# tusen-ai/SST

Hardware: AMD Instinct MI355X
Metric: LiDAR frames/sec (SST backbone fwd+bwd) at Waymo 0.32m voxels (higher is better)
Workload: dtype f32 (storage, accumulation, attention, LayerNorm, reductions: fp32; the dense products of the encoder layers from the EXACT three-way bf16 split of both fp32 operands, six bf16 MFMA products with fp32 accumulation - error vs float64 <= 2 x the fp32 matrix pipe's: tests/test_gpu_dense_f32x6.py)

## Files before the change

sst_amd/csrc/dense_f32x6.hip:

```cpp
#include <math.h>
#include <stdlib.h>
#include "common.h"
#include "tile_io.h"

namespace {

typedef float f32x4 __attribute__((ext_vector_type(4)));
typedef float f32x2 __attribute__((ext_vector_type(2)));
typedef unsigned u32x4 __attribute__((ext_vector_type(4)));
typedef __bf16 bf16x8 __attribute__((ext_vector_type(8)));
typedef __bf16 bf16x2 __attribute__((ext_vector_type(2)));

__device__ __forceinline__ unsigned pack2(float lo, float hi) {
  const f32x2 v = {lo, hi};
  return __builtin_bit_cast(unsigned, __builtin_convertvector(v, bf16x2));
}
__device__ __forceinline__ float lo_f(unsigned p) { return __uint_as_float(p << 16); }
__device__ __forceinline__ float hi_f(unsigned p) { return __uint_as_float(p & 0xffff0000u); }
__device__ __forceinline__ f32x4 mma32(u32x4 a, u32x4 b, f32x4 c) {
  return __builtin_amdgcn_mfma_f32_16x16x32_bf16(__builtin_bit_cast(bf16x8, a), __builtin_bit_cast(bf16x8, b), c, 0, 0, 0);
}
__device__ __forceinline__ void split2(float a, float b, unsigned& p0, unsigned& p1, unsigned& p2) {
  p0 = pack2(a, b);
  const float ra = a - lo_f(p0), rb = b - hi_f(p0);
// ... 3 lines not shown
__device__ __forceinline__ void split8(const f32x4& a, const f32x4& b, u32x4& p0, u32x4& p1, u32x4& p2) {
  unsigned q0[4], q1[4], q2[4];
  split2(a[0], a[1], q0[0], q1[0], q2[0]);
  split2(a[2], a[3], q0[1], q1[1], q2[1]);
  split2(b[0], b[1], q0[2], q1[2], q2[2]);
  split2(b[2], b[3], q0[3], q1[3], q2[3]);
  p0 = (u32x4){q0[0], q0[1], q0[2], q0[3]};
  p1 = (u32x4){q1[0], q1[1], q1[2], q1[3]};
  p2 = (u32x4){q2[0], q2[1], q2[2], q2[3]};
}

__device__ __forceinline__ float erf_as(float z, float& e) {
  const float az = fabsf(z);
  const float t = __builtin_amdgcn_rcpf(fmaf(0.3275911f, az, 1.f));
  e = __expf(-az * az);
  const float poly = t * fmaf(t, fmaf(t, fmaf(t, fmaf(t, 1.061405429f, -1.453152027f), 1.421413741f), -0.284496736f), 0.254829592f);
  return copysignf(fmaf(-poly, e, 1.f), z);
}
__device__ __forceinline__ float gelu_f(float x) {
  float e;
  return 0.5f * x * (1.f + erf_as(x * 0.70710678118654752f, e));
}
__device__ __forceinline__ float gelu_grad_f(float x) {
  float e;
  const float phi = 0.5f * (1.f + erf_as(x * 0.70710678118654752f, e));
  return fmaf(x * 0.3989422804014327f, e, phi);
}

enum { kEpiBias = 0, kEpiGelu = 1, kEpiRelu = 2, kEpiMulGeluGrad = 3, kEpiMulReluGrad = 4, kEpiAdd = 5, kEpiAddLN = 6,
       kEpiAddRows = 7 };

struct ln_epi {
  const float* w;
  const float* b;
  float eps;
  float2* stats;
  const float* pos_table;
  const int32_t* pos_idx;
  float* yp;
};

__device__ __forceinline__ int w_lds_row(int n) {
  const int tp = n >> 5, within = n & 31;
  return 16 * (2 * tp + ((within >> 2) & 1)) + ((within >> 3) << 2) + (within & 3);
}

template <int K, int NW, int EPI>
constexpr bool x6_bias_in_regs() {
  return 3 * NW * K * 2 + NW * (EPI == kEpiAddLN ? 3 : 1) * 4 + 8 * 2048 > 160 * 1024;
}
template <int K, int NW, int EPI>
constexpr int x6_lds_bytes() {
  return 3 * NW * K * 2 + (x6_bias_in_regs<K, NW, EPI>() ? 0 : NW * (EPI == kEpiAddLN ? 3 : 1) * 4) + 8 * 2048;
}

template <int K, int NW, int EPI, bool XADD = false>
__global__ __launch_bounds__(512, 2) void tall_linear_f32x6_k(
    const float* __restrict__ X, const float* __restrict__ X2, int x2_from, int64_t ldx, const float* __restrict__ W,
    int64_t ldw, int trans_w, const float* __restrict__ bias, int64_t M, int row_blocks, int rows_per_wave,
    float* __restrict__ Y, int64_t ldy, const float* __restrict__ aux_in, float* __restrict__ aux_out, int64_t ldaux,
    const ln_epi ln, const float* __restrict__ xadd_rows = nullptr, const int32_t* __restrict__ xadd_idx = nullptr) {
  static_assert(EPI != kEpiAddLN || NW == 128, "the LayerNorm epilogue needs a whole 128-wide row in one accumulator set");
  static_assert(NW == 64 || NW == 128, "column group");
  constexpr int KS = K / 32, NTH = 512, TILES = NW / 16, EMITS = TILES / 2;
  constexpr int IMG = NW * K * 2;
  constexpr bool BIAS_REG = x6_bias_in_regs<K, NW, EPI>();
  constexpr bool HAS_AUX = EPI == kEpiMulGeluGrad || EPI == kEpiMulReluGrad || EPI == kEpiAdd || EPI == kEpiAddLN || EPI == kEpiAddRows;
  static_assert(!(BIAS_REG && EPI == kEpiAddLN), "the LayerNorm epilogue reads its row parameters from LDS");
  extern __shared__ __attribute__((aligned(16))) unsigned char smem6[];
  unsigned char* w0 = smem6;
  unsigned char* w1 = smem6 + IMG;
  unsigned char* w2 = smem6 + 2 * IMG;
  float* bimg = (float*)(smem6 + 3 * IMG);
  auto frag_off = [](int lr, int k8) { return ((lr >> 4) * KS + (k8 >> 5)) * 1024 + (16 * ((k8 >> 3) & 3) + (lr & 15)) * 16; };
  const int lane = threadIdx.x & 63, g = lane >> 4, c = lane & 15;
  const int wv = __builtin_amdgcn_readfirstlane(threadIdx.x >> 6);
  const int rr = lane >> 3, rcol = (lane & 7) * 4;
  const tile_xpose io =
      make_tile_xpose(smem6 + 3 * IMG + (BIAS_REG ? 0 : NW * (EPI == kEpiAddLN ? 3 : 1) * 4) + wv * 2048, lane);
  const int grp = blockIdx.x / row_blocks, rb = blockIdx.x - grp * row_blocks;
  const int nb = grp * NW;
  const float* __restrict__ Xg = grp >= x2_from ? X2 : X;
  const int64_t wave = (int64_t)rb * 8 + wv;
  int64_t r0 = wave * rows_per_wave;
  const int64_t r1 = r0 + rows_per_wave < M ? r0 + rows_per_wave : M;
  auto row_of = [&](int64_t r, int i) {
    const int64_t row = r + 8 * i + rr;
    return row < M ? row : M - 1;
  };
  constexpr int D = EPI == kEpiAddLN ? 2 : (KS > 8 ? KS / 2 : KS);
  static_assert(!XADD || D == KS, "the positional rows of a tile are requested with one set of indices");
  static_assert(KS % D == 0, "a block keeps its slot from tile to tile");
  f32x4 xr[D][2];
  auto issue_x = [&](int64_t r, int s) {
#pragma unroll
    for (int i = 0; i < 2; ++i) xr[s % D][i] = *(const f32x4*)(Xg + row_of(r, i) * ldx + 32 * s + rcol);
  };
  const bool xadd = XADD && grp < x2_from;
  f32x4 pr[XADD ? D : 1][2];
  int32_t pi[2] = {0, 0};
  auto load_pidx = [&](int64_t r, int32_t (&dst)[2]) {
#pragma unroll
    for (int i = 0; i < 2; ++i) dst[i] = xadd_idx[row_of(r, i)];
  };
  auto issue_p = [&](int s) {
#pragma unroll
// ... 138 lines not shown
            pend[T][r] -= mean;
            sq = fmaf(pend[T][r], pend[T][r], sq);
          }
        sq += __shfl_xor(sq, 16, 64);
        sq += __shfl_xor(sq, 32, 64);
        ln_rstd = rsqrtf(sq * (1.f / 128.f) + ln.eps);
        if (g == 0 && pend_r0 + c < M) ln.stats[pend_r0 + c] = make_float2(mean, ln_rstd);
      }
      const int n0 = 32 * tp + 8 * g;
      const f32x4 y0 = pend[2 * tp] * ln_rstd * *(const f32x4*)(bimg + NW + n0) + *(const f32x4*)(bimg + 2 * NW + n0);
      const f32x4 y1 =
          pend[2 * tp + 1] * ln_rstd * *(const f32x4*)(bimg + NW + n0 + 4) + *(const f32x4*)(bimg + 2 * NW + n0 + 4);
      f32x4 t[2];
      tile_to_rows(io, y0, y1, t[0], t[1]);
#pragma unroll
      for (int i = 0; i < 2; ++i)
        if (pv[i]) *(f32x4*)(Y + prow[i] * ldy + 32 * tp + rcol) = t[i];
      if (gather) {
#pragma unroll
        for (int i = 0; i < 2; ++i)
          if (pv[i]) *(f32x4*)(ln.yp + prow[i] * 128 + 32 * tp + rcol) = t[i] + qr[i];
      }
      return;
    }
    const int n0 = nb + 32 * tp + rcol;
    const f32x4 bv = BIAS_REG ? breg[BIAS_REG ? tp : 0] : *(const f32x4*)(bimg + 32 * tp + rcol);
    f32x4 t[2];
    tile_to_rows(io, pend[2 * tp], pend[2 * tp + 1], t[0], t[1]);
#pragma unroll
    for (int i = 0; i < 2; ++i) {
      f32x4 v = t[i] + bv;
      if (EPI == kEpiGelu || EPI == kEpiRelu) {
        if (aux_out != nullptr && pv[i]) *(f32x4*)(aux_out + prow[i] * ldaux + n0) = v;
#pragma unroll
        for (int r = 0; r < 4; ++r) v[r] = EPI == kEpiGelu ? gelu_f(v[r]) : fmaxf(v[r], 0.f);
      }
      if (EPI == kEpiMulGeluGrad || EPI == kEpiMulReluGrad) {
        const f32x4 p = ar[HAS_AUX ? tp : 0][i];
#pragma unroll
        for (int r = 0; r < 4; ++r) v[r] *= EPI == kEpiMulGeluGrad ? gelu_grad_f(p[r]) : (p[r] > 0.f ? 1.f : 0.f);
      }
      if (EPI == kEpiAdd || EPI == kEpiAddRows) v += ar[HAS_AUX ? tp : 0][i];
      if (pv[i]) *(f32x4*)(Y + prow[i] * ldy + n0) = v;
    }
  };
  auto emit = [&](int tp, bool in_loop) {
    if (pend_valid) consume(tp);
    if (in_loop)
      request(tp);
    else if (EPI == kEpiAddLN && gather && tp + 1 < EMITS)
      issue_q(ep, tp + 1);
  };

  for (; r0 < r1; r0 += 16) {
    asm volatile("" ::: "memory");
    const int64_t rn = r0 + 16 < r1 ? r0 + 16 : r0;
    int32_t pj[2] = {0, 0};
    if (xadd) load_pidx(r0 + 32, pj);
    if (GATHER && gather) load_eidx(r0 + 16, en);
    f32x4 acc[TILES];
#pragma unroll
    for (int T = 0; T < TILES; ++T) acc[T] = (f32x4){0.f, 0.f, 0.f, 0.f};
    constexpr int QPS = TILES / 4;
    constexpr int G = KS * QPS;
    u32x4 x0, x1, x2;
#pragma clang loop unroll(full)
    for (int q = 0; q < G; ++q) {
      const int s = q / QPS, t0 = (q % QPS) * 4;
      if (q % QPS == 0) {
        f32x4 a = xr[s % D][0], b = xr[s % D][1];
        if (XADD && xadd) {
          a += pr[XADD ? s % D : 0][0];
          b += pr[XADD ? s % D : 0][1];
        }
        f32x4 v0, v1;
        tile_to_frag(io, a, b, v0, v1);
        split8(v0, v1, x0, x1, x2);
        if (s + D < KS) {
          issue_x(r0, s + D);
        } else {
          issue_x(rn, s + D - KS);
          if (XADD && xadd) issue_p(s + D - KS);
        }
        __builtin_amdgcn_sched_barrier(0x786);
      }
      u32x4 a0[4], a1[4], a2[4];
#pragma unroll
      for (int u = 0; u < 4; ++u) {
        const int off = lane_off + ((t0 + u) * KS + s) * 1024;
        a0[u] = *(const u32x4*)(w0 + off);
        a1[u] = *(const u32x4*)(w1 + off);
        a2[u] = *(const u32x4*)(w2 + off);
      }
#pragma unroll
      for (int u = 0; u < 4; ++u) acc[t0 + u] = mma32(a0[u], x2, acc[t0 + u]);
#pragma unroll
      for (int u = 0; u < 4; ++u) acc[t0 + u] = mma32(a2[u], x0, acc[t0 + u]);
#pragma unroll
      for (int u = 0; u < 4; ++u) acc[t0 + u] = mma32(a1[u], x1, acc[t0 + u]);
#pragma unroll
      for (int u = 0; u < 4; ++u) acc[t0 + u] = mma32(a0[u], x1, acc[t0 + u]);
#pragma unroll
      for (int u = 0; u < 4; ++u) acc[t0 + u] = mma32(a1[u], x0, acc[t0 + u]);
#pragma unroll
      for (int u = 0; u < 4; ++u) acc[t0 + u] = mma32(a0[u], x0, acc[t0 + u]);
      if ((q + 1) % (G / EMITS) == 0) emit((q + 1) / (G / EMITS) - 1, true);
    }
#pragma unroll
    for (int T = 0; T < TILES; ++T) pend[T] = acc[T];
    pend_r0 = r0;
    pend_valid = true;
#pragma unroll
    for (int i = 0; i < 2; ++i) {
      pi[i] = pj[i];
      ep[i] = ec[i];
      ec[i] = en[i];
    }
  }
#pragma unroll
  for (int tp = 0; tp < EMITS; ++tp) emit(tp, false);
}

void x6_partition(int64_t m, int groups, int64_t& row_blocks, int64_t& rpw) {
  row_blocks = (256 / groups) & ~7;
  rpw = sst_align_up(sst_div_up(m, row_blocks * 8), 16);
  row_blocks = sst_align_up(sst_div_up(m, rpw * 8), 8);
}

template <int K, int NW, int EPI, bool XADD = false>
int launch_x6(const float* x, const float* x2, int x2_from, int64_t ldx, const float* w, int64_t ldw, int trans_w,
              const float* bias, int64_t m, int n, float* y, int64_t ldy, const float* aux_in, float* aux_out, int64_t ldaux,
              hipStream_t st, const ln_epi ln = ln_epi(), const float* xadd_rows = nullptr, const int32_t* xadd_idx = nullptr) {
  constexpr int lds = x6_lds_bytes<K, NW, EPI>();
  static_assert(lds <= 160 * 1024, "three weight images of a column group and the waves' blocks must fit the CU's LDS");
  static unsigned long long configured = 0;
  if (sst_first_use_on_device(&configured)) {
    SST_HIP(hipFuncSetAttribute((const void*)tall_linear_f32x6_k<K, NW, EPI, XADD>, hipFuncAttributeMaxDynamicSharedMemorySize, lds));
    sst_mark_device(&configured);
  }
  const int groups = n / NW;
  int64_t row_blocks, rpw;
  x6_partition(m, groups, row_blocks, rpw);
  if (x2 == nullptr) x2_from = groups;
  hipLaunchKernelGGL((tall_linear_f32x6_k<K, NW, EPI, XADD>), dim3((unsigned)(row_blocks * groups)), dim3(512), lds, st, x, x2,
                     x2_from, ldx, w, ldw, trans_w, bias, m, (int)row_blocks, (int)rpw, y, ldy, aux_in, aux_out, ldaux, ln, xadd_rows,
                     xadd_idx);
  return SST_OK;
}

template <int K, int NW>
int dispatch_x6(int epi, const float* x, const float* x2, int x2_from, int64_t ldx, const float* w, int64_t ldw, int trans_w,
                const float* bias, int64_t m, int n, float* y, int64_t ldy, const float* aux_in, float* aux_out, int64_t ldaux,
                hipStream_t st) {
#define SST_CASE(E) \
  case E: return launch_x6<K, NW, E>(x, x2, x2_from, ldx, w, ldw, trans_w, bias, m, n, y, ldy, aux_in, aux_out, ldaux, st)
  switch (epi) {
    SST_CASE(kEpiBias);
    SST_CASE(kEpiGelu);
    SST_CASE(kEpiRelu);
// ... 131 lines not shown
```

sst_amd/csrc/layer_tail_x6.hip:

```cpp
#include <math.h>
#include <stdlib.h>
#include "common.h"

#ifndef SST_NT_OUT
#define SST_NT_OUT false
#endif
#ifndef SST_NT_BWD
#define SST_NT_BWD true
#endif

namespace {

typedef float f32x4 __attribute__((ext_vector_type(4)));
typedef float f32x2 __attribute__((ext_vector_type(2)));
typedef unsigned u32x4 __attribute__((ext_vector_type(4)));
typedef __bf16 bf16x8 __attribute__((ext_vector_type(8)));
typedef __bf16 bf16x2 __attribute__((ext_vector_type(2)));

__device__ __forceinline__ unsigned pack2(float lo, float hi) {
  const f32x2 v = {lo, hi};
  return __builtin_bit_cast(unsigned, __builtin_convertvector(v, bf16x2));
}
__device__ __forceinline__ float lo_f(unsigned p) { return __uint_as_float(p << 16); }
__device__ __forceinline__ float hi_f(unsigned p) { return __uint_as_float(p & 0xffff0000u); }
// ... 206 lines not shown
__device__ __forceinline__ void barrier_lds_only() { asm volatile("s_waitcnt lgkmcnt(0)\n\ts_barrier" ::: "memory"); }
__device__ __forceinline__ void barrier_drain() { asm volatile("s_waitcnt vmcnt(0) lgkmcnt(0)\n\ts_barrier" ::: "memory"); }

struct tile_io {
  unsigned char* scr;
  int frag_off0;
  int row_off[2];
  int64_t rrow[2];
  bool rvalid[2];
  int rcol;
};
__device__ __forceinline__ tile_io make_tile_io(unsigned char* scr, int lane, int64_t r0, int64_t m) {
  tile_io t;
  const int c = lane & 15, g = lane >> 4;
  t.scr = scr;
  t.frag_off0 = c * 128 + (((2 * g) ^ (c & 7)) << 4);
#pragma unroll
  for (int i = 0; i < 2; ++i) {
    const int r = 8 * i + (lane >> 3), p = lane & 7;
    t.row_off[i] = r * 128 + ((p ^ (r & 7)) << 4);
    t.rvalid[i] = r0 + r < m;
    t.rrow[i] = t.rvalid[i] ? r0 + r : m - 1;
  }
  t.rcol = (lane & 7) * 4;
  return t;
}
template <bool STREAM>
__device__ __forceinline__ void store32(const tile_io& t, float* __restrict__ base, int64_t ld, int col0, const f32x4& v0,
                                        const f32x4& v1) {
  *(f32x4*)(t.scr + t.frag_off0) = v0;
  *(f32x4*)(t.scr + (t.frag_off0 ^ 16)) = v1;
#pragma unroll
  for (int i = 0; i < 2; ++i) {
    const f32x4 w = *(const f32x4*)(t.scr + t.row_off[i]);
    if (t.rvalid[i]) {
      if (STREAM)
        __builtin_nontemporal_store(w, (f32x4*)(base + t.rrow[i] * ld + col0 + t.rcol));
      else
        *(f32x4*)(base + t.rrow[i] * ld + col0 + t.rcol) = w;
    }
  }
}
__device__ __forceinline__ void load32_issue(const tile_io& t, const float* __restrict__ base, int64_t ld, int col0, f32x4 (&w)[2]) {
#pragma unroll
  for (int i = 0; i < 2; ++i) w[i] = *(const f32x4*)(base + t.rrow[i] * ld + col0 + t.rcol);
}
__device__ __forceinline__ void load32_finish(const tile_io& t, const f32x4 (&w)[2], f32x4& v0, f32x4& v1) {
#pragma unroll
  for (int i = 0; i < 2; ++i) *(f32x4*)(t.scr + t.row_off[i]) = w[i];
  v0 = *(const f32x4*)(t.scr + t.frag_off0);
  v1 = *(const f32x4*)(t.scr + (t.frag_off0 ^ 16));
}

template <int HALF>
__device__ __forceinline__ void mma_half(const unsigned char* slot, int lane_off, const f32x4 (&x)[4][2], f32x4 (&acc)[8]) {
#pragma unroll
  for (int s2 = 0; s2 < 2; ++s2) {
    const img3 xs = split8(x[2 * HALF + s2][0], x[2 * HALF + s2][1]);
#pragma unroll
    for (int t0 = 0; t0 < 8; t0 += 4) {
      u32x4 a0[4], a1[4], a2[4];
#pragma unroll
      for (int u = 0; u < 4; ++u) {
        const int off = lane_off + ((t0 + u) * 2 + s2) * kFrag;
        a0[u] = *(const u32x4*)(slot + off);
        a1[u] = *(const u32x4*)(slot + kIA + off);
        a2[u] = *(const u32x4*)(slot + 2 * kIA + off);
      }
#pragma unroll
      for (int u = 0; u < 4; ++u) acc[t0 + u] = mma32(a0[u], xs.p2, acc[t0 + u]);
#pragma unroll
      for (int u = 0; u < 4; ++u) acc[t0 + u] = mma32(a2[u], xs.p0, acc[t0 + u]);
#pragma unroll
      for (int u = 0; u < 4; ++u) acc[t0 + u] = mma32(a1[u], xs.p1, acc[t0 + u]);
#pragma unroll
      for (int u = 0; u < 4; ++u) acc[t0 + u] = mma32(a0[u], xs.p1, acc[t0 + u]);
#pragma unroll
      for (int u = 0; u < 4; ++u) acc[t0 + u] = mma32(a1[u], xs.p0, acc[t0 + u]);
#pragma unroll
      for (int u = 0; u < 4; ++u) acc[t0 + u] = mma32(a0[u], xs.p0, acc[t0 + u]);
    }
  }
}

__device__ __forceinline__ f32x4 add4(const f32x4& a, const f32x4& b) {
  return (f32x4){a[0] + b[0], a[1] + b[1], a[2] + b[2], a[3] + b[3]};
}

__device__ __forceinline__ void mma_first(const unsigned char* slot, int lane_off1, const img3 (&y)[4], f32x4& out0, f32x4& out1) {
  const f32x4 z = {0.f, 0.f, 0.f, 0.f};
  f32x4 am[2] = {z, z}, ca[2] = {z, z}, cb[2] = {z, z};
#pragma unroll
  for (int s = 0; s < 4; ++s) {
    u32x4 a0[2], a1[2], a2[2];
#pragma unroll
    for (int T = 0; T < 2; ++T) {
      const int off = lane_off1 + (T * 4 + s) * kFrag;
      a0[T] = *(const u32x4*)(slot + off);
      a1[T] = *(const u32x4*)(slot + kI1 + off);
      a2[T] = *(const u32x4*)(slot + 2 * kI1 + off);
    }
#pragma unroll
    for (int T = 0; T < 2; ++T) ca[T] = mma32(a0[T], y[s].p2, ca[T]);
#pragma unroll
    for (int T = 0; T < 2; ++T) cb[T] = mma32(a0[T], y[s].p1, cb[T]);
#pragma unroll
    for (int T = 0; T < 2; ++T) ca[T] = mma32(a2[T], y[s].p0, ca[T]);
#pragma unroll
    for (int T = 0; T < 2; ++T) am[T] = mma32(a0[T], y[s].p0, am[T]);
#pragma unroll
    for (int T = 0; T < 2; ++T) ca[T] = mma32(a1[T], y[s].p1, ca[T]);
#pragma unroll
    for (int T = 0; T < 2; ++T) cb[T] = mma32(a1[T], y[s].p0, cb[T]);
  }
  out0 = add4(am[0], add4(cb[0], ca[0]));
  out1 = add4(am[1], add4(cb[1], ca[1]));
}

__device__ __forceinline__ void mma_second(const unsigned char* slot2, int lane_off2, const img3& h, f32x4 (&acc)[8]) {
#pragma unroll
  for (int t0 = 0; t0 < 8; t0 += 4) {
    u32x4 a0[4], a1[4], a2[4];
#pragma unroll
    for (int u = 0; u < 4; ++u) {
      const int off = lane_off2 + (t0 + u) * kFrag;
      a0[u] = *(const u32x4*)(slot2 + off);
      a1[u] = *(const u32x4*)(slot2 + kI2 + off);
      a2[u] = *(const u32x4*)(slot2 + 2 * kI2 + off);
    }
#pragma unroll
    for (int u = 0; u < 4; ++u) acc[t0 + u] = mma32(a0[u], h.p2, acc[t0 + u]);
#pragma unroll
    for (int u = 0; u < 4; ++u) acc[t0 + u] = mma32(a2[u], h.p0, acc[t0 + u]);
#pragma unroll
    for (int u = 0; u < 4; ++u) acc[t0 + u] = mma32(a1[u], h.p1, acc[t0 + u]);
#pragma unroll
    for (int u = 0; u < 4; ++u) acc[t0 + u] = mma32(a0[u], h.p1, acc[t0 + u]);
#pragma unroll
    for (int u = 0; u < 4; ++u) acc[t0 + u] = mma32(a1[u], h.p0, acc[t0 + u]);
#pragma unroll
    for (int u = 0; u < 4; ++u) acc[t0 + u] = mma32(a0[u], h.p0, acc[t0 + u]);
  }
}

__device__ __forceinline__ void ln_stats(f32x4 (&v)[4][2], float eps, float& mean, float& rstd) {
  float sum = 0.f;
#pragma unroll
  for (int s = 0; s < 4; ++s)
#pragma unroll
    for (int r = 0; r < 4; ++r) sum += v[s][0][r] + v[s][1][r];
  sum += __shfl_xor(sum, 16, 64);
  sum += __shfl_xor(sum, 32, 64);
  mean = sum * (1.f / 128.f);
  float sq = 0.f;
#pragma unroll
  for (int s = 0; s < 4; ++s)
#pragma unroll
    for (int h = 0; h < 2; ++h)
#pragma unroll
      for (int r = 0; r < 4; ++r) {
        v[s][h][r] -= mean;
        sq = fmaf(v[s][h][r], v[s][h][r], sq);
      }
  sq += __shfl_xor(sq, 16, 64);
  sq += __shfl_xor(sq, 32, 64);
  rstd = rsqrtf(sq * (1.f / 128.f) + eps);
}

struct tail_fwd_params {
  const float *o, *x;
  const unsigned char* packed;
  const float *b_out, *b1, *b2, *n1w, *n1b, *n2w, *n2b;
  float eps;
  int64_t m;
  float *s1, *st1, *y1, *pre, *h, *s2, *st2, *y2;
  const float* pos_table;
  const int32_t* pos_idx;
  float* y2p;
};

template <int ACT>
__global__ __launch_bounds__(kNTH, 2) void encoder_tail_fwd_x6_k(const tail_fwd_params P) {
  extern __shared__ __attribute__((aligned(16))) unsigned char lds[];
  float* par = (float*)(lds + kArea);
  const int lane = threadIdx.x & 63, g = lane >> 4, c = lane & 15, wave = threadIdx.x >> 6;
  const int64_t r0 = (int64_t)blockIdx.x * kRowsPerWg + wave * 16;
  const bool valid = r0 + c < P.m;
  const int64_t row = valid ? r0 + c : P.m - 1;
  const tile_io io = make_tile_io(lds + kArea + kParF * 4 + wave * kScr, lane, r0, P.m);
  const unsigned char* packed = P.packed;
  unsigned char* const part2 = lds + kPart1;
  dma_pieces(packed, lds, 3 * kIA / 1024, wave, lane);
  f32x4 ob[4][2], xr[4][2];
  {
    f32x4 wo[4][2], wx[4][2];
#pragma unroll
    for (int s = 0; s < 4; ++s) load32_issue(io, P.o, kC, 32 * s, wo[s]);
#pragma unroll
    for (int s = 0; s < 4; ++s) load32_issue(io, P.x, kC, 32 * s, wx[s]);
#pragma unroll
    for (int s = 0; s < 4; ++s) load32_finish(io, wo[s], ob[s][0], ob[s][1]);
#pragma unroll
    for (int s = 0; s < 4; ++s) load32_finish(io, wx[s], xr[s][0], xr[s][1]);
  }
  for (int i = threadIdx.x; i < kC; i += kNTH) {
    par[i] = P.b_out ? P.b_out[i] : 0.f;
    par[kC + i] = P.n1w[i];
    par[2 * kC + i] = P.n1b[i];
    par[3 * kC + i] = P.b2 ? P.b2[i] : 0.f;
    par[4 * kC + i] = P.n2w[i];
    par[5 * kC + i] = P.n2b[i];
  }
  for (int i = threadIdx.x; i < kFF; i += kNTH) par[6 * kC + i] = P.b1 ? P.b1[i] : 0.f;

  const int lane_offA = lane * 16, lane_off1 = lane * 16, lane_off2 = lane * 16;
  const f32x4 z4 = {0.f, 0.f, 0.f, 0.f};
  f32x4 acc[8];
#pragma unroll
  for (int T = 0; T < 8; ++T) acc[T] = z4;
  img3 yi[4];

  barrier_drain();
  mma_half<0>(lds, lane_offA, ob, acc);
  barrier_drain();
  dma_pieces(packed + kSlot, lds, 3 * kIA / 1024, wave, lane);
  barrier_drain();
  mma_half<1>(lds, lane_offA, ob, acc);
  barrier_drain();
  dma_pieces(packed + 2 * kSlot, lds, kSlot / 1024, wave, lane);
  {
    f32x4 v[4][2];
#pragma unroll
    for (int s = 0; s < 4; ++s) {
      const int n0 = 32 * s + 8 * g;
      v[s][0] = acc[2 * s] + *(const f32x4*)(par + n0) + xr[s][0];
      v[s][1] = acc[2 * s + 1] + *(const f32x4*)(par + n0 + 4) + xr[s][1];
      if (P.s1 != nullptr) store32<true>(io, P.s1, kC, 32 * s, v[s][0], v[s][1]);
    }
    float mean, rstd;
    ln_stats(v, P.eps, mean, rstd);
    if (valid && g == 0) ((float2*)P.st1)[row] = make_float2(mean, rstd);
#pragma unroll
    for (int s = 0; s < 4; ++s) {
      const int n0 = 32 * s + 8 * g;
      const f32x4 y0 = v[s][0] * rstd * *(const f32x4*)(par + kC + n0) + *(const f32x4*)(par + 2 * kC + n0);
      const f32x4 y1 = v[s][1] * rstd * *(const f32x4*)(par + kC + n0 + 4) + *(const f32x4*)(par + 2 * kC + n0 + 4);
      store32<true>(io, P.y1, kC, 32 * s, y0, y1);
      yi[s] = split8(y0, y1);
    }
#pragma unroll
    for (int T = 0; T < 8; ++T) acc[T] = z4;
  }
  barrier_drain();
  f32x4 sp0 = z4, sp1 = z4, sh0 = z4, sh1 = z4;
#pragma unroll 1
  for (int j = 0; j < kNF; ++j) {
    if (j > 0) {
      store32<true>(io, P.pre, kFF, kHC * (j - 1), sp0, sp1);
      store32<true>(io, P.h, kFF, kHC * (j - 1), sh0, sh1);
    }
    f32x4 p0, p1;
    mma_first(lds, lane_off1, yi, p0, p1);
    const int nl = kHC * j + 8 * g;
    p0 = add4(p0, *(const f32x4*)(par + 6 * kC + nl));
    p1 = add4(p1, *(const f32x4*)(par + 6 * kC + nl + 4));
    f32x4 h0, h1;
#pragma unroll
    for (int r = 0; r < 4; ++r) {
      h0[r] = ACT == 1 ? gelu_f(p0[r]) : fmaxf(p0[r], 0.f);
      h1[r] = ACT == 1 ? gelu_f(p1[r]) : fmaxf(p1[r], 0.f);
    }
    const img3 hs = split8(h0, h1);
    barrier_drain();
    if (j + 1 < kNF) dma_pieces(packed + (size_t)(j + 3) * kSlot, lds, kPart1 / 1024, wave, lane);
    mma_second(part2, lane_off2, hs, acc);
    sp0 = p0, sp1 = p1, sh0 = h0, sh1 = h1;
    barrier_drain();
    if (j + 1 < kNF) dma_pieces(packed + (size_t)(j + 3) * kSlot + kPart1, part2, kPart2 / 1024, wave, lane);
  }
  store32<true>(io, P.pre, kFF, kHC * (kNF - 1), sp0, sp1);
  store32<true>(io, P.h, kFF, kHC * (kNF - 1), sh0, sh1);
  f32x4 v[4][2];
#pragma unroll
  for (int s = 0; s < 4; ++s) {
    const int n0 = 32 * s + 8 * g;
    f32x4 ya, yb;
    join8(yi[s], ya, yb);
    v[s][0] = acc[2 * s] + *(const f32x4*)(par + 3 * kC + n0) + ya;
    v[s][1] = acc[2 * s + 1] + *(const f32x4*)(par + 3 * kC + n0 + 4) + yb;
    if (P.s2 != nullptr) store32<true>(io, P.s2, kC, 32 * s, v[s][0], v[s][1]);
  }
  float mean, rstd;
  ln_stats(v, P.eps, mean, rstd);
  if (valid && g == 0) ((float2*)P.st2)[row] = make_float2(mean, rstd);
  const float* prow = P.pos_table != nullptr ? P.pos_table + (size_t)P.pos_idx[row] * kC : nullptr;
#pragma unroll
  for (int s = 0; s < 4; ++s) {
    const int n0 = 32 * s + 8 * g;
    const f32x4 y0 = v[s][0] * rstd * *(const f32x4*)(par + 4 * kC + n0) + *(const f32x4*)(par + 5 * kC + n0);
    const f32x4 y1 = v[s][1] * rstd * *(const f32x4*)(par + 4 * kC + n0 + 4) + *(const f32x4*)(par + 5 * kC + n0 + 4);
    store32<SST_NT_OUT>(io, P.y2, kC, 32 * s, y0, y1);
    if (prow != nullptr) store32<SST_NT_OUT>(io, P.y2p, kC, 32 * s, y0 + *(const f32x4*)(prow + n0), y1 + *(const f32x4*)(prow + n0 + 4));
  }
}

struct tail_bwd_params {
  const float *dy2, *dy2p, *s2, *st2, *n2w, *pre, *s1, *st1, *n1w;
  const unsigned char* packed;
  int64_t m;
  float *ds2, *dpre, *ds1, *d_o;
  float *part2, *part1;
};

__device__ __forceinline__ void ln_bwd(f32x4 (&d)[4][2], f32x4 (&sv)[4][2], const float2 st, const float* gamma, int g, int c,
                                       bool valid, float* red) {
  float sg = 0.f, sgx = 0.f;
#pragma unroll
  for (int s = 0; s < 4; ++s)
#pragma unroll
    for (int h = 0; h < 2; ++h) {
      const f32x4 w = *(const f32x4*)(gamma + 32 * s + 8 * g + 4 * h);
      sv[s][h] = (sv[s][h] - st.x) * st.y;
      f32x4 a, b;
#pragma unroll
      for (int r = 0; r < 4; ++r) {
        a[r] = row_sum16(valid ? d[s][h][r] * sv[s][h][r] : 0.f);
        b[r] = row_sum16(valid ? d[s][h][r] : 0.f);
      }
// ... 34 lines not shown
  const unsigned char* packed = P.packed;
  unsigned char* const part2 = lds + kPart1;
  dma_pieces(packed, lds, kSlot / 1024, wave, lane);
  f32x4 d[4][2], sv[4][2];
  {
    f32x4 wd[4][2], we[4][2];
#pragma unroll
    for (int s = 0; s < 4; ++s) load32_issue(io, P.dy2, kC, 32 * s, wd[s]);
    if (P.dy2p != nullptr) {
#pragma unroll
      for (int s = 0; s < 4; ++s) load32_issue(io, P.dy2p, kC, 32 * s, we[s]);
#pragma unroll
      for (int s = 0; s < 4; ++s) {
        wd[s][0] += we[s][0];
        wd[s][1] += we[s][1];
      }
    }
#pragma unroll
    for (int s = 0; s < 4; ++s) load32_issue(io, P.s2, kC, 32 * s, we[s]);
#pragma unroll
    for (int s = 0; s < 4; ++s) load32_finish(io, wd[s], d[s][0], d[s][1]);
#pragma unroll
    for (int s = 0; s < 4; ++s) load32_finish(io, we[s], sv[s][0], sv[s][1]);
  }
  const float2 st2 = ((const float2*)P.st2)[row];
  for (int i = threadIdx.x; i < kC; i += kNTH) {
    par[i] = P.n2w[i];
    par[kC + i] = P.n1w[i];
  }
  barrier_drain();

  img3 di[4];
  {
    ln_bwd(d, sv, st2, par, g, c, valid, red + wave * 2 * kC);
#pragma unroll
    for (int s = 0; s < 4; ++s) {
      store32<SST_NT_BWD>(io, P.ds2, kC, 32 * s, d[s][0], d[s][1]);
      di[s] = split8(d[s][0], d[s][1]);
    }
  }
  const int lane_offA = lane * 16, lane_off1 = lane * 16, lane_off2 = lane * 16;
  const f32x4 z4 = {0.f, 0.f, 0.f, 0.f};
  f32x4 acc[8];
#pragma unroll
  for (int T = 0; T < 8; ++T) acc[T] = z4;
  f32x4 xs1[4][2];
  f32x4 pq[2];
  load32_issue(io, P.pre, kFF, 0, pq);

  f32x4 sd0 = z4, sd1 = z4;
  auto ffn_chunk = [&](int j, const f32x4 q0, const f32x4 q1) __attribute__((always_inline)) {
    if (j > 0) store32<SST_NT_BWD>(io, P.dpre, kFF, kHC * (j - 1), sd0, sd1);
    f32x4 p0, p1;
    mma_first(lds, lane_off1, di, p0, p1);
#pragma unroll
    for (int r = 0; r < 4; ++r) {
      p0[r] *= ACT == 1 ? gelu_grad_f(q0[r]) : (q0[r] > 0.f ? 1.f : 0.f);
      p1[r] *= ACT == 1 ? gelu_grad_f(q1[r]) : (q1[r] > 0.f ? 1.f : 0.f);
    }
    const img3 hs = split8(p0, p1);
    barrier_drain();
    if (j + 1 < kNF) dma_pieces(packed + (size_t)(j + 1) * kSlot, lds, kPart1 / 1024, wave, lane);
    mma_second(part2, lane_off2, hs, acc);
    sd0 = p0, sd1 = p1;
    barrier_drain();
    if (j + 1 < kNF)
      dma_pieces(packed + (size_t)(j + 1) * kSlot + kPart1, part2, kPart2 / 1024, wave, lane);
    else
      dma_pieces(packed + (size_t)kNF * kSlot, lds, 3 * kIA / 1024, wave, lane);
  };
  barrier_drain();
  if (threadIdx.x < 2 * kC) {
    float a = 0.f;
#pragma unroll
    for (int w = 0; w < kWaves; ++w) a += red[w * 2 * kC + threadIdx.x];
    P.part2[(int64_t)blockIdx.x * 2 * kC + threadIdx.x] = a;
  }
#pragma unroll 1
  for (int j = 0; j < kNF - 1; ++j) {
    f32x4 q0, q1;
    load32_finish(io, pq, q0, q1);
    load32_issue(io, P.pre, kFF, kHC * (j + 1), pq);
    ffn_chunk(j, q0, q1);
  }
  {
    f32x4 q0, q1;
    load32_finish(io, pq, q0, q1);
    ffn_chunk(kNF - 1, q0, q1);
    store32<SST_NT_BWD>(io, P.dpre, kFF, kHC * (kNF - 1), sd0, sd1);
    {
      f32x4 ws[4][2];
#pragma unroll
      for (int s = 0; s < 4; ++s) load32_issue(io, P.s1, kC, 32 * s, ws[s]);
#pragma unroll
      for (int s = 0; s < 4; ++s) load32_finish(io, ws[s], xs1[s][0], xs1[s][1]);
    }
    f32x4 dd[4][2];
#pragma unroll
    for (int s = 0; s < 4; ++s) {
      f32x4 ya, yb;
      join8(di[s], ya, yb);
      dd[s][0] = acc[2 * s] + ya;
      dd[s][1] = acc[2 * s + 1] + yb;
    }
    const float2 st1 = ((const float2*)P.st1)[row];
    barrier_drain();
    ln_bwd(dd, xs1, st1, par + kC, g, c, valid, red + wave * 2 * kC);
#pragma unroll
    for (int s = 0; s < 4; ++s) {
      store32<SST_NT_BWD>(io, P.ds1, kC, 32 * s, dd[s][0], dd[s][1]);
      xs1[s][0] = dd[s][0];
      xs1[s][1] = dd[s][1];
    }
#pragma unroll
    for (int T = 0; T < 8; ++T) acc[T] = z4;
    barrier_drain();
    mma_half<0>(lds, lane_offA, xs1, acc);
    barrier_drain();
    dma_pieces(packed + (size_t)(kNF + 1) * kSlot, lds, 3 * kIA / 1024, wave, lane);
    barrier_drain();
    mma_half<1>(lds, lane_offA, xs1, acc);
  }
#pragma unroll
  for (int s = 0; s < 4; ++s) store32<SST_NT_OUT>(io, P.d_o, kC, 32 * s, acc[2 * s], acc[2 * s + 1]);
  barrier_drain();
  if (threadIdx.x < 2 * kC) {
    float b = 0.f;
#pragma unroll
    for (int w = 0; w < kWaves; ++w) b += red[w * 2 * kC + threadIdx.x];
    P.part1[(int64_t)blockIdx.x * 2 * kC + threadIdx.x] = b;
  }
}

bool aligned16(const void* p) { return ((uintptr_t)p & 15) == 0; }

template <typename K>
int configure(K kernel, int lds_bytes, unsigned long long* mask) {
  if (sst_first_use_on_device(mask)) {
    SST_HIP(hipFuncSetAttribute((const void*)kernel, hipFuncAttributeMaxDynamicSharedMemorySize, lds_bytes));
    sst_mark_device(mask);
  }
  return SST_OK;
}

}

int sst_internal_encoder_tail_bwd_f32x6(const sst_encoder_tail_bwd_args* a, float** part2, float** part1, int* partial_rows,
                                        void* stream) {
  if (!a || a->m <= 0 || (a->act != 1 && a->act != 2)) return SST_ERR_ARG;
  const void* need[] = {a->dy2, a->s2, a->st2, a->n2w, a->pre, a->s1, a->st1, a->n1w, a->packed,
                        a->ds2, a->dpre, a->ds1, a->d_o, a->workspace};
  for (const void* p : need)
    if (!p || !aligned16(p)) return SST_ERR_ARG;
  if (a->dy2p && !aligned16(a->dy2p)) return SST_ERR_ARG;
  const int64_t rows = sst_div_up(a->m, (int64_t)kRowsPerWg);
  if (rows > 0x7fffffff / 2) return SST_ERR_UNSUPPORTED;
  tail_bwd_params P;
  P.dy2 = a->dy2, P.dy2p = a->dy2p, P.s2 = a->s2, P.st2 = a->st2, P.n2w = a->n2w, P.pre = a->pre, P.s1 = a->s1, P.st1 = a->st1;
  P.n1w = a->n1w, P.packed = (const unsigned char*)a->packed + kPackDir, P.m = a->m;
  P.ds2 = a->ds2, P.dpre = a->dpre, P.ds1 = a->ds1, P.d_o = a->d_o;
  P.part2 = (float*)a->workspace;
  P.part1 = P.part2 + rows * 2 * kC;
  hipStream_t st = (hipStream_t)stream;
  static unsigned long long cfg1 = 0, cfg2 = 0;
  if (a->act == 1) {
    const int rc = configure(encoder_tail_bwd_x6_k<1>, kLdsBwd, &cfg1);
    if (rc) return rc;
    hipLaunchKernelGGL(encoder_tail_bwd_x6_k<1>, dim3((unsigned)rows), dim3(kNTH), kLdsBwd, st, P);
  } else {
    const int rc = configure(encoder_tail_bwd_x6_k<2>, kLdsBwd, &cfg2);
    if (rc) return rc;
    hipLaunchKernelGGL(encoder_tail_bwd_x6_k<2>, dim3((unsigned)rows), dim3(kNTH), kLdsBwd, st, P);
  }
  SST_LAUNCH_CHECK();
// ... 114 lines not shown
```

Baseline: 100.6.

## Software-pipeline LDS weight fragment loads across MFMA groups with pinned scheduling

Adds a streaming path for the f32x6 dense and layer-tail kernels. Each group's weight fragments for the next column group are loaded from LDS while the current group's six bf16 MFMA products run, using a double-buffered hi-part fragment set and sched_group_barrier pinning so ds_reads interleave with MFMAs. In the dense kernel, the next activation block's split and issue is also moved ahead. This should hide LDS read latency behind the matrix pipe, at the cost of more VGPRs and a fragile hand-written schedule. The path is enabled by default, except for the LayerNorm epilogue and positional-add variants.

New measurement: 100.2. About the same (-0.5%).

```diff
diff --git a/sst_amd/csrc/dense_f32x6.hip b/sst_amd/csrc/dense_f32x6.hip
--- a/sst_amd/csrc/dense_f32x6.hip
+++ b/sst_amd/csrc/dense_f32x6.hip
@@ -79,6 +79,36 @@
 template <int K, int NW, int EPI>
 constexpr int x6_lds_bytes() {
   return 3 * NW * K * 2 + (x6_bias_in_regs<K, NW, EPI>() ? 0 : NW * (EPI == kEpiAddLN ? 3 : 1) * 4) + 8 * 2048;
+}
+
+#ifndef SST_X6_FRAG_STREAM
+#define SST_X6_FRAG_STREAM 1
+#endif
+template <int K, int NW, int EPI, bool XADD>
+constexpr bool x6_frag_stream() {
+  return SST_X6_FRAG_STREAM != 0 && EPI != kEpiAddLN && !XADD;
+}
+__device__ __forceinline__ void x6_pin_head() {
+#pragma unroll
+  for (int u = 0; u < 4; ++u) {
+    __builtin_amdgcn_sched_group_barrier(0x100, 1, 0);
+    __builtin_amdgcn_sched_group_barrier(0x8, 1, 0);
+  }
+  __builtin_amdgcn_sched_group_barrier(0x8, 4, 0);
+#pragma unroll
+  for (int u = 0; u < 2; ++u) {
+    __builtin_amdgcn_sched_group_barrier(0x100, 2, 0);
+    __builtin_amdgcn_sched_group_barrier(0x8, 1, 0);
+  }
+  __builtin_amdgcn_sched_group_barrier(0x8, 10, 0);
+}
+__device__ __forceinline__ void x6_pin_tail() {
+#pragma unroll
+  for (int u = 0; u < 2; ++u) {
+    __builtin_amdgcn_sched_group_barrier(0x100, 2, 0);
+    __builtin_amdgcn_sched_group_barrier(0x8, 1, 0);
+  }
+  __builtin_amdgcn_sched_group_barrier(0x8, 2, 0);
 }
 
 template <int K, int NW, int EPI, bool XADD = false>
@@ -323,6 +353,31 @@
       issue_q(ep, tp + 1);
   };
 
+  constexpr int QPS = TILES / 4;
+  constexpr int G = KS * QPS;
+  constexpr bool STREAM = x6_frag_stream<K, NW, EPI, XADD>();
+  static_assert(!STREAM || G % 2 == 0, "the fragment sets rotate with period 2");
+  auto frag_at = [&](int q, int u) { return lane_off + (((q % QPS) * 4 + u) * KS + q / QPS) * 1024; };
+  u32x4 fa0[2][4], fa1[4], fa2[4];
+  if (STREAM) {
+#pragma unroll
+    for (int u = 0; u < 4; ++u) {
+      fa0[0][u] = *(const u32x4*)(w0 + frag_at(0, u));
+      fa1[u] = *(const u32x4*)(w1 + frag_at(0, u));
+      fa2[u] = *(const u32x4*)(w2 + frag_at(0, u));
+    }
+  }
+  static_assert(!(STREAM && XADD), "the positional rows are added in the old placement only");
+  f32x4 v0n, v1n;
+  auto next_block = [&](int s, int64_t rt, int64_t rtn) {
+    tile_to_frag(io, xr[s % D][0], xr[s % D][1], v0n, v1n);
+    if (s + D < KS)
+      issue_x(rt, s + D);
+    else
+      issue_x(rtn, s + D - KS);
+  };
+  if (STREAM) next_block(0, r0, r0 + 16 < r1 ? r0 + 16 : r0);
+
   for (; r0 < r1; r0 += 16) {
     asm volatile("" ::: "memory");
     const int64_t rn = r0 + 16 < r1 ? r0 + 16 : r0;
@@ -332,13 +387,12 @@
     f32x4 acc[TILES];
 #pragma unroll
     for (int T = 0; T < TILES; ++T) acc[T] = (f32x4){0.f, 0.f, 0.f, 0.f};
-    constexpr int QPS = TILES / 4;
-    constexpr int G = KS * QPS;
     u32x4 x0, x1, x2;
 #pragma clang loop unroll(full)
     for (int q = 0; q < G; ++q) {
       const int s = q / QPS, t0 = (q % QPS) * 4;
-      if (q % QPS == 0) {
+      if (STREAM && q % QPS == 0) split8(v0n, v1n, x0, x1, x2);
+      if (!STREAM && q % QPS == 0) {
         f32x4 a = xr[s % D][0], b = xr[s % D][1];
         if (XADD && xadd) {
           a += pr[XADD ? s % D : 0][0];
@@ -355,27 +409,61 @@
         }
         __builtin_amdgcn_sched_barrier(0x786);
       }
-      u32x4 a0[4], a1[4], a2[4];
-#pragma unroll
-      for (int u = 0; u < 4; ++u) {
-        const int off = lane_off + ((t0 + u) * KS + s) * 1024;
-        a0[u] = *(const u32x4*)(w0 + off);
-        a1[u] = *(const u32x4*)(w1 + off);
-        a2[u] = *(const u32x4*)(w2 + off);
-      }
-#pragma unroll
-      for (int u = 0; u < 4; ++u) acc[t0 + u] = mma32(a0[u], x2, acc[t0 + u]);
-#pragma unroll
-      for (int u = 0; u < 4; ++u) acc[t0 + u] = mma32(a2[u], x0, acc[t0 + u]);
-#pragma unroll
-      for (int u = 0; u < 4; ++u) acc[t0 + u] = mma32(a1[u], x1, acc[t0 + u]);
-#pragma unroll
-      for (int u = 0; u < 4; ++u) acc[t0 + u] = mma32(a0[u], x1, acc[t0 + u]);
-#pragma unroll
-      for (int u = 0; u < 4; ++u) acc[t0 + u] = mma32(a1[u], x0, acc[t0 + u]);
-#pragma unroll
-      for (int u = 0; u < 4; ++u) acc[t0 + u] = mma32(a0[u], x0, acc[t0 + u]);
-      if ((q + 1) % (G / EMITS) == 0) emit((q + 1) / (G / EMITS) - 1, true);
+      if (STREAM) {
+        const int cur = q & 1, nq = (q + 1) % G;
+#pragma unroll
+        for (int u = 0; u < 4; ++u) fa0[cur ^ 1][u] = *(const u32x4*)(w0 + frag_at(nq, u));
+#pragma unroll
+        for (int u = 0; u < 4; ++u) acc[t0 + u] = mma32(fa0[cur][u], x2, acc[t0 + u]);
+#pragma unroll
+        for (int u = 0; u < 4; ++u) acc[t0 + u] = mma32(fa2[u], x0, acc[t0 + u]);
+#pragma unroll
+        for (int u = 0; u < 4; ++u) fa2[u] = *(const u32x4*)(w2 + frag_at(nq, u));
+#pragma unroll
+        for (int u = 0; u < 4; ++u) acc[t0 + u] = mma32(fa1[u], x1, acc[t0 + u]);
+#pragma unroll
+        for (int u = 0; u < 4; ++u) acc[t0 + u] = mma32(fa0[cur][u], x1, acc[t0 + u]);
+#pragma unroll
+        for (int u = 0; u < 4; ++u) acc[t0 + u] = mma32(fa1[u], x0, acc[t0 + u]);
+        x6_pin_head();
+        const bool last_of_kstep = (q + 1) % QPS == 0, emits = (q + 1) % (G / EMITS) == 0;
+        if (last_of_kstep || emits) __builtin_amdgcn_sched_barrier(0);
+        if (last_of_kstep) {
+          if (s + 1 < KS)
+            next_block(s + 1, r0, rn);
+          else
+            next_block(0, rn, rn + 16 < r1 ? rn + 16 : rn);
+        }
+        if (emits) emit((q + 1) / (G / EMITS) - 1, true);
+        if (last_of_kstep || emits) __builtin_amdgcn_sched_barrier(0);
+#pragma unroll
+        for (int u = 0; u < 4; ++u) fa1[u] = *(const u32x4*)(w1 + frag_at(nq, u));
+#pragma unroll
+        for (int u = 0; u < 4; ++u) acc[t0 + u] = mma32(fa0[cur][u], x0, acc[t0 + u]);
+        x6_pin_tail();
+      } else {
+        u32x4 a0[4], a1[4], a2[4];
+#pragma unroll
+        for (int u = 0; u < 4; ++u) {
+          const int off = frag_at(q, u);
+          a0[u] = *(const u32x4*)(w0 + off);
+          a1[u] = *(const u32x4*)(w1 + off);
+          a2[u] = *(const u32x4*)(w2 + off);
+        }
+#pragma unroll
+        for (int u = 0; u < 4; ++u) acc[t0 + u] = mma32(a0[u], x2, acc[t0 + u]);
+#pragma unroll
+        for (int u = 0; u < 4; ++u) acc[t0 + u] = mma32(a2[u], x0, acc[t0 + u]);
+#pragma unroll
+        for (int u = 0; u < 4; ++u) acc[t0 + u] = mma32(a1[u], x1, acc[t0 + u]);
+#pragma unroll
+        for (int u = 0; u < 4; ++u) acc[t0 + u] = mma32(a0[u], x1, acc[t0 + u]);
+#pragma unroll
+        for (int u = 0; u < 4; ++u) acc[t0 + u] = mma32(a1[u], x0, acc[t0 + u]);
+#pragma unroll
+        for (int u = 0; u < 4; ++u) acc[t0 + u] = mma32(a0[u], x0, acc[t0 + u]);
+      }
+      if (!STREAM && (q + 1) % (G / EMITS) == 0) emit((q + 1) / (G / EMITS) - 1, true);
     }
 #pragma unroll
     for (int T = 0; T < TILES; ++T) pend[T] = acc[T];
diff --git a/sst_amd/csrc/layer_tail_x6.hip b/sst_amd/csrc/layer_tail_x6.hip
--- a/sst_amd/csrc/layer_tail_x6.hip
+++ b/sst_amd/csrc/layer_tail_x6.hip
@@ -282,8 +282,89 @@
   v1 = *(const f32x4*)(t.scr + (t.frag_off0 ^ 16));
 }
 
-template <int HALF>
+#ifndef SST_X6_FRAG_STREAM
+#define SST_X6_FRAG_STREAM 1
+#endif
+constexpr bool kStreamFwd = SST_X6_FRAG_STREAM != 0;
+constexpr bool kStreamBwd = SST_X6_FRAG_STREAM != 0;
+
+template <int NG, typename OFF, typename XS>
+__device__ __forceinline__ void mma_groups_stream(const unsigned char* base, int img, OFF off, XS xs, f32x4 (&acc)[8]) {
+  u32x4 a0[2][4], a1[4], a2[4];
+  __builtin_amdgcn_sched_barrier(0);
+#pragma unroll
+  for (int u = 0; u < 4; ++u) {
+    a0[0][u] = *(const u32x4*)(base + off(0, u));
+    a2[u] = *(const u32x4*)(base + 2 * img + off(0, u));
+    a1[u] = *(const u32x4*)(base + img + off(0, u));
+  }
+  __builtin_amdgcn_sched_group_barrier(0x100, 12, 0);
+#pragma unroll
+  for (int gi = 0; gi < NG; ++gi) {
+    const int cur = gi & 1, t0 = (gi * 4) & 7;
+    const bool more = gi + 1 < NG;
+    const img3 x = xs(gi);
+    if (more) {
+#pragma unroll
+      for (int u = 0; u < 4; ++u) a0[cur ^ 1][u] = *(const u32x4*)(base + off(gi + 1, u));
+    }
+#pragma unroll
+    for (int u = 0; u < 4; ++u) acc[t0 + u] = mma32(a0[cur][u], x.p2, acc[t0 + u]);
+#pragma unroll
+    for (int u = 0; u < 4; ++u) acc[t0 + u] = mma32(a2[u], x.p0, acc[t0 + u]);
+    if (more) {
+#pragma unroll
+      for (int u = 0; u < 4; ++u) a2[u] = *(const u32x4*)(base + 2 * img + off(gi + 1, u));
+    }
+#pragma unroll
+    for (int u = 0; u < 4; ++u) acc[t0 + u] = mma32(a1[u], x.p1, acc[t0 + u]);
+#pragma unroll
+    for (int u = 0; u < 4; ++u) acc[t0 + u] = mma32(a0[cur][u], x.p1, acc[t0 + u]);
+#pragma unroll
+    for (int u = 0; u < 4; ++u) acc[t0 + u] = mma32(a1[u], x.p0, acc[t0 + u]);
+    if (more) {
+#pragma unroll
+      for (int u = 0; u < 4; ++u) a1[u] = *(const u32x4*)(base + img + off(gi + 1, u));
+    }
+#pragma unroll
+    for (int u = 0; u < 4; ++u) acc[t0 + u] = mma32(a0[cur][u], x.p0, acc[t0 + u]);
+    if (more) {
+#pragma unroll
+      for (int u = 0; u < 4; ++u) {
+        __builtin_amdgcn_sched_group_barrier(0x100, 1, 0);
+        __builtin_amdgcn_sched_group_barrier(0x8, 1, 0);
+      }
+      __builtin_amdgcn_sched_group_barrier(0x8, 4, 0);
+#pragma unroll
+      for (int u = 0; u < 2; ++u) {
+        __builtin_amdgcn_sched_group_barrier(0x100, 2, 0);
+        __builtin_amdgcn_sched_group_barrier(0x8, 1, 0);
+      }
+      __builtin_amdgcn_sched_group_barrier(0x8, 10, 0);
+#pragma unroll
+      for (int u = 0; u < 2; ++u) {
+        __builtin_amdgcn_sched_group_barrier(0x100, 2, 0);
+        __builtin_amdgcn_sched_group_barrier(0x8, 1, 0);
+      }
+      __builtin_amdgcn_sched_group_barrier(0x8, 2, 0);
+    }
+  }
+  __builtin_amdgcn_sched_barrier(0);
+}
+
+template <int HALF, bool STREAM>
 __device__ __forceinline__ void mma_half(const unsigned char* slot, int lane_off, const f32x4 (&x)[4][2], f32x4 (&acc)[8]) {
+  if (STREAM) {
+    img3 xk[2];
+    mma_groups_stream<4>(
+        slot, kIA, [&](int gi, int u) { return lane_off + (((gi & 1) * 4 + u) * 2 + (gi >> 1)) * kFrag; },
+        [&](int gi) {
+          if ((gi & 1) == 0) xk[gi >> 1] = split8(x[2 * HALF + (gi >> 1)][0], x[2 * HALF + (gi >> 1)][1]);
+          return xk[gi >> 1];
+        },
+        acc);
+    return;
+  }
 #pragma unroll
   for (int s2 = 0; s2 < 2; ++s2) {
     const img3 xs = split8(x[2 * HALF + s2][0], x[2 * HALF + s2][1]);
@@ -317,37 +398,88 @@
   return (f32x4){a[0] + b[0], a[1] + b[1], a[2] + b[2], a[3] + b[3]};
 }
 
+template <bool STREAM>
 __device__ __forceinline__ void mma_first(const unsigned char* slot, int lane_off1, const img3 (&y)[4], f32x4& out0, f32x4& out1) {
   const f32x4 z = {0.f, 0.f, 0.f, 0.f};
   f32x4 am[2] = {z, z}, ca[2] = {z, z}, cb[2] = {z, z};
-#pragma unroll
-  for (int s = 0; s < 4; ++s) {
-    u32x4 a0[2], a1[2], a2[2];
+  if (STREAM) {
+    u32x4 a0[2][2], a1[2], a2[2];
+    __builtin_amdgcn_sched_barrier(0);
 #pragma unroll
     for (int T = 0; T < 2; ++T) {
-      const int off = lane_off1 + (T * 4 + s) * kFrag;
-      a0[T] = *(const u32x4*)(slot + off);
-      a1[T] = *(const u32x4*)(slot + kI1 + off);
-      a2[T] = *(const u32x4*)(slot + 2 * kI1 + off);
-    }
-#pragma unroll
-    for (int T = 0; T < 2; ++T) ca[T] = mma32(a0[T], y[s].p2, ca[T]);
-#pragma unroll
-    for (int T = 0; T < 2; ++T) cb[T] = mma32(a0[T], y[s].p1, cb[T]);
-#pragma unroll
-    for (int T = 0; T < 2; ++T) ca[T] = mma32(a2[T], y[s].p0, ca[T]);
-#pragma unroll
-    for (int T = 0; T < 2; ++T) am[T] = mma32(a0[T], y[s].p0, am[T]);
-#pragma unroll
-    for (int T = 0; T < 2; ++T) ca[T] = mma32(a1[T], y[s].p1, ca[T]);
-#pragma unroll
-    for (int T = 0; T < 2; ++T) cb[T] = mma32(a1[T], y[s].p0, cb[T]);
+      a0[0][T] = *(const u32x4*)(slot + lane_off1 + (T * 4) * kFrag);
+      a2[T] = *(const u32x4*)(slot + 2 * kI1 + lane_off1 + (T * 4) * kFrag);
+    }
+    __builtin_amdgcn_sched_group_barrier(0x100, 4, 0);
+#pragma unroll
+    for (int s = 0; s < 4; ++s) {
+      const int cur = s & 1;
+      const bool more = s + 1 < 4;
+#pragma unroll
+      for (int T = 0; T < 2; ++T) a1[T] = *(const u32x4*)(slot + kI1 + lane_off1 + (T * 4 + s) * kFrag);
+      if (more) {
+#pragma unroll
+        for (int T = 0; T < 2; ++T) a0[cur ^ 1][T] = *(const u32x4*)(slot + lane_off1 + (T * 4 + s + 1) * kFrag);
+      }
+#pragma unroll
+      for (int T = 0; T < 2; ++T) ca[T] = mma32(a0[cur][T], y[s].p2, ca[T]);
+#pragma unroll
+      for (int T = 0; T < 2; ++T) cb[T] = mma32(a0[cur][T], y[s].p1, cb[T]);
+#pragma unroll
+      for (int T = 0; T < 2; ++T) ca[T] = mma32(a2[T], y[s].p0, ca[T]);
+      if (more) {
+#pragma unroll
+        for (int T = 0; T < 2; ++T) a2[T] = *(const u32x4*)(slot + 2 * kI1 + lane_off1 + (T * 4 + s + 1) * kFrag);
+      }
+#pragma unroll
+      for (int T = 0; T < 2; ++T) am[T] = mma32(a0[cur][T], y[s].p0, am[T]);
+#pragma unroll
+      for (int T = 0; T < 2; ++T) ca[T] = mma32(a1[T], y[s].p1, ca[T]);
+#pragma unroll
+      for (int T = 0; T < 2; ++T) cb[T] = mma32(a1[T], y[s].p0, cb[T]);
+      __builtin_amdgcn_sched_group_barrier(0x100, 2, 0);
+      if (more) __builtin_amdgcn_sched_group_barrier(0x100, 2, 0);
+      __builtin_amdgcn_sched_group_barrier(0x8, 6, 0);
+      if (more) __builtin_amdgcn_sched_group_barrier(0x100, 2, 0);
+      __builtin_amdgcn_sched_group_barrier(0x8, 6, 0);
+    }
+    __builtin_amdgcn_sched_barrier(0);
+  } else {
+#pragma unroll
+    for (int s = 0; s < 4; ++s) {
+      u32x4 a0[2], a1[2], a2[2];
+#pragma unroll
+      for (int T = 0; T < 2; ++T) {
+        const int off = lane_off1 + (T * 4 + s) * kFrag;
+        a0[T] = *(const u32x4*)(slot + off);
+        a1[T] = *(const u32x4*)(slot + kI1 + off);
+        a2[T] = *(const u32x4*)(slot + 2 * kI1 + off);
+      }
+#pragma unroll
+      for (int T = 0; T < 2; ++T) ca[T] = mma32(a0[T], y[s].p2, ca[T]);
+#pragma unroll
+      for (int T = 0; T < 2; ++T) cb[T] = mma32(a0[T], y[s].p1, cb[T]);
+#pragma unroll
+      for (int T = 0; T < 2; ++T) ca[T] = mma32(a2[T], y[s].p0, ca[T]);
+#pragma unroll
+      for (int T = 0; T < 2; ++T) am[T] = mma32(a0[T], y[s].p0, am[T]);
+#pragma unroll
+      for (int T = 0; T < 2; ++T) ca[T] = mma32(a1[T], y[s].p1, ca[T]);
+#pragma unroll
+      for (int T = 0; T < 2; ++T) cb[T] = mma32(a1[T], y[s].p0, cb[T]);
+    }
   }
   out0 = add4(am[0], add4(cb[0], ca[0]));
   out1 = add4(am[1], add4(cb[1], ca[1]));
 }
 
+template <bool STREAM>
 __device__ __forceinline__ void mma_second(const unsigned char* slot2, int lane_off2, const img3& h, f32x4 (&acc)[8]) {
+  if (STREAM) {
+    mma_groups_stream<2>(
+        slot2, kI2, [&](int gi, int u) { return lane_off2 + (gi * 4 + u) * kFrag; }, [&](int) { return h; }, acc);
+    return;
+  }
 #pragma unroll
   for (int t0 = 0; t0 < 8; t0 += 4) {
     u32x4 a0[4], a1[4], a2[4];
@@ -451,11 +583,11 @@
   img3 yi[4];
 
   barrier_drain();
-  mma_half<0>(lds, lane_offA, ob, acc);
+  mma_half<0, kStreamFwd>(lds, lane_offA, ob, acc);
   barrier_drain();
   dma_pieces(packed + kSlot, lds, 3 * kIA / 1024, wave, lane);
   barrier_drain();
-  mma_half<1>(lds, lane_offA, ob, acc);
+  mma_half<1, kStreamFwd>(lds, lane_offA, ob, acc);
   barrier_drain();
   dma_pieces(packed + 2 * kSlot, lds, kSlot / 1024, wave, lane);
   {
@@ -490,7 +622,7 @@
       store32<true>(io, P.h, kFF, kHC * (j - 1), sh0, sh1);
     }
     f32x4 p0, p1;
-    mma_first(lds, lane_off1, yi, p0, p1);
+    mma_first<kStreamFwd>(lds, lane_off1, yi, p0, p1);
     const int nl = kHC * j + 8 * g;
     p0 = add4(p0, *(const f32x4*)(par + 6 * kC + nl));
     p1 = add4(p1, *(const f32x4*)(par + 6 * kC + nl + 4));
@@ -503,7 +635,7 @@
     const img3 hs = split8(h0, h1);
     barrier_drain();
     if (j + 1 < kNF) dma_pieces(packed + (size_t)(j + 3) * kSlot, lds, kPart1 / 1024, wave, lane);
-    mma_second(part2, lane_off2, hs, acc);
+    mma_second<kStreamFwd>(part2, lane_off2, hs, acc);
     sp0 = p0, sp1 = p1, sh0 = h0, sh1 = h1;
     barrier_drain();
     if (j + 1 < kNF) dma_pieces(packed + (size_t)(j + 3) * kSlot + kPart1, part2, kPart2 / 1024, wave, lane);
@@ -644,7 +776,7 @@
   auto ffn_chunk = [&](int j, const f32x4 q0, const f32x4 q1) __attribute__((always_inline)) {
     if (j > 0) store32<SST_NT_BWD>(io, P.dpre, kFF, kHC * (j - 1), sd0, sd1);
     f32x4 p0, p1;
-    mma_first(lds, lane_off1, di, p0, p1);
+    mma_first<kStreamBwd>(lds, lane_off1, di, p0, p1);
 #pragma unroll
     for (int r = 0; r < 4; ++r) {
       p0[r] *= ACT == 1 ? gelu_grad_f(q0[r]) : (q0[r] > 0.f ? 1.f : 0.f);
@@ -653,7 +785,7 @@
     const img3 hs = split8(p0, p1);
     barrier_drain();
     if (j + 1 < kNF) dma_pieces(packed + (size_t)(j + 1) * kSlot, lds, kPart1 / 1024, wave, lane);
-    mma_second(part2, lane_off2, hs, acc);
+    mma_second<kStreamBwd>(part2, lane_off2, hs, acc);
     sd0 = p0, sd1 = p1;
     barrier_drain();
     if (j + 1 < kNF)
@@ -707,11 +839,11 @@
 #pragma unroll
     for (int T = 0; T < 8; ++T) acc[T] = z4;
     barrier_drain();
-    mma_half<0>(lds, lane_offA, xs1, acc);
+    mma_half<0, kStreamBwd>(lds, lane_offA, xs1, acc);
     barrier_drain();
     dma_pieces(packed + (size_t)(kNF + 1) * kSlot, lds, 3 * kIA / 1024, wave, lane);
     barrier_drain();
-    mma_half<1>(lds, lane_offA, xs1, acc);
+    mma_half<1, kStreamBwd>(lds, lane_offA, xs1, acc);
   }
 #pragma unroll
   for (int s = 0; s < 4; ++s) store32<SST_NT_OUT>(io, P.d_o, kC, 32 * s, acc[2 * s], acc[2 * s + 1]);
```
